# lxjeffffff/PagedAttention-Based-Transformer-Decoder-Inference-Framework

Hardware: AMD Instinct MI355X
Metric: decode tokens/sec at batch=64 seq_len=8192; % HBM-roofline (1/2/4/8 GPU) (higher is better)
Workload: dtype int8 GEMM (i32 acc) + fp16 KV attention (fp32 acc); 1 GPU; C3: INT8 decoder (MFMA i8 matmuls + fp16 paged attention), 24-layer/16-head/d=128, batch 64, KV context 8192, page 16; strong scaling: 64 rows over 1 GPU(s); global_batch=64, batch_per_gpu=64, seq_len=8192, page_size=16, parallelism=single GPU (no collective)

## Files before the change

pagedattention-based-transformer-decoder-inference-framework_amd/csrc/gemm_impl.hpp:

```cpp
#pragma once

#include "common.hpp"
#include "fp8.hpp"
#include "gemm.hpp"
#include "ln_wave.hpp"

namespace llm {

struct KvAppend {
  const int32_t* pos;
  const int32_t* page_table;
  const int32_t* rows;
  _Float16* k_pool;
  _Float16* v_pool;
  int num_beams, max_tiles, TS, num_pages, H, D;
  size_t page_stride;
  int fp8;
  float k_inv, v_inv;
};

struct GemmArgs {
  const uint8_t* A;
  int lda;
  int a_packed;
  const uint8_t* B;
  int M, N, K, KS;
  const float* sa;
  const float* sw;
  const float* bias;
  int act;
  float* C;
  int32_t* acc_out;
  int c_cols;
  int c_ld;
  _Float16* c16;
  KvAppend kv;
  unsigned long long* stamps;
  const float* ln_x;
  const _Float16* ln_emb;
  const int32_t* ln_tok;
  int ln_V;
  const float* ln_g;
  const float* ln_b;
  float ln_eps;
  uint8_t* act_out;
  float* sa_out;
  int partial;
  int w_keep;
  int xcd_map;
  unsigned* seam;
  int seam_n;
  int qdiag;
  int ksplit2;
};

__host__ __device__ constexpr int ln_row_stride(int K, int esize) { return K * esize + 32; }

__device__ __forceinline__ unsigned long long phase_clock() {
  unsigned long long t;
  asm volatile("s_memrealtime %0\n\ts_waitcnt lgkmcnt(0)" : "=s"(t)::"memory");
  return t;
}


template <int MT, int WAVES, int NT = 1>
constexpr int gemm_unroll() {
  return (MT >= 4 ? 2 : 4) * (WAVES == 4 ? 2 : 1) / (NT >= 4 ? 2 : 1);
}

__device__ __forceinline__ float apply_act(float y, int act) {
  if (act == LLM_ACT_RELU) return fmaxf(y, 0.f);
  if (act == LLM_ACT_GELU) return 0.5f * y * (1.f + erff(y * 0.70710678118654752f));
  return y;
}

enum class GemmKind { I8, F16 };

template <GemmKind KIND>
struct GemmTraits;
template <>
struct GemmTraits<GemmKind::I8> {
  static constexpr int KSTEP = 64, ESIZE = 1;
  using acc_t = i32x4;
  using elem_t = int32_t;
};
template <>
struct GemmTraits<GemmKind::F16> {
  static constexpr int KSTEP = 32, ESIZE = 2;
  using acc_t = f32x4;
  using elem_t = float;
};

template <GemmKind KIND, int ROWS, int WAVES>
__device__ __forceinline__ void ln_prologue(const GemmArgs& a, int m0, uint8_t* alds,
                                            float* sa_lds) {
  constexpr int ESIZE = GemmTraits<KIND>::ESIZE;
  constexpr int CPL = 8;
  const int lane = lane_id();
  const int w = wave_id_uniform();
  const int K = a.K;
  const int K4 = K >> 2;
  const int stride = ln_row_stride(K, ESIZE);
  const bool do_ln = a.ln_g != nullptr;
  LnRow<CPL> gm, bt;
  ln_wave_load(a.ln_g, K4, do_ln, gm);
  ln_wave_load(a.ln_b, K4, do_ln, bt);
  for (int r0 = w; r0 < ROWS; r0 += 2 * WAVES) {
    LnRow<CPL> x[2];
#pragma unroll
    for (int q = 0; q < 2; ++q) {
      const int r = r0 + q * WAVES;
      const int m = m0 + r;
      const bool ok = r < ROWS && m < a.M;
      if (a.ln_emb)
        ln_wave_load_f16(ok ? ln_embed_row(a.ln_emb, a.ln_tok, m, a.ln_V, K) : a.ln_emb, K4, ok,
// ... 5 lines not shown
    for (int q = 0; q < 2; ++q) {
      const int r = r0 + q * WAVES;
      if (r >= ROWS) break;
      const bool mok = m0 + r < a.M;
      float am;
      if (do_ln) {
        am = ln_wave_compute(x[q], gm, bt, K, a.ln_eps);
      } else {
        am = 0.f;
#pragma unroll
        for (int j = 0; j < CPL; ++j)
#pragma unroll
          for (int e = 0; e < 4; ++e) am = fmaxf(am, fabsf(x[q].v[j][e]));
        am = ln_wave_max(am);
      }
      uint8_t* rowp = alds + (size_t)r * stride;
      if constexpr (KIND == GemmKind::I8) {
        const float scale = 127.f / (am + 1e-6f);
#pragma unroll
        for (int j = 0; j < CPL; ++j) {
          const int c = 64 * j + lane;
          if (c < K4)
            *reinterpret_cast<uint32_t*>(rowp + 4 * c) = mok ? ln_quant4(x[q].v[j], scale) : 0u;
        }
        if (lane == 0) sa_lds[r] = mok ? 1.0f / scale : 0.f;
      } else {
#pragma unroll
        for (int j = 0; j < CPL; ++j) {
          const int c = 64 * j + lane;
          if (c < K4)
            *reinterpret_cast<ln_f16x4*>(rowp + 8 * c) =
                mok ? ln_half4(x[q].v[j]) : ln_f16x4{0, 0, 0, 0};
        }
      }
    }
  }
}

__device__ __forceinline__ void seam_wait(unsigned* ctr, int n) {
  if (threadIdx.x == 0) {
    unsigned spins = 0;
    while (__hip_atomic_load(&ctr[0], __ATOMIC_RELAXED, __HIP_MEMORY_SCOPE_AGENT) < (unsigned)n) {
      __builtin_amdgcn_s_sleep(8);
      if (++spins > (1u << 21)) {
        __hip_atomic_store(&ctr[2], 1u, __ATOMIC_RELAXED, __HIP_MEMORY_SCOPE_AGENT);
        break;
      }
    }
    __builtin_amdgcn_fence(__ATOMIC_ACQUIRE, "agent");
  }
  __syncthreads();
}

template <GemmKind KIND, int MT, int NT, int WAVES, int DIAG = 0, int PRO = 0, int SEAM = 0>
__device__ __forceinline__ void gemm_tile(const GemmArgs& a, int bx, int by, int bz, int nz,
                                          int gx) {
  using Tr = GemmTraits<KIND>;
  using acc_t = typename Tr::acc_t;
  constexpr int KSTEP = Tr::KSTEP;
  constexpr int kUnroll = gemm_unroll<MT, WAVES, NT>();
  using elem_t = typename Tr::elem_t;
  using RedT = elem_t[MT * NT][4][64];
  extern __shared__ __attribute__((aligned(16))) uint8_t gemm_smem[];
  RedT* red;
  if constexpr (PRO == 0) {
    __shared__ elem_t red_static[WAVES][MT * NT][4][64];
    red = red_static;
  } else {
    red = reinterpret_cast<RedT*>(gemm_smem);
  }
  constexpr int ROWS_ = 16 * MT;
  const int a_stride = ln_row_stride(a.K, Tr::ESIZE);
  uint8_t* alds = gemm_smem;
  float* sa_lds = reinterpret_cast<float*>(gemm_smem + (size_t)ROWS_ * a_stride);

  const int lane = lane_id();
  const int w = wave_id_uniform();
  const int nt0 = bx * NT;
  const int m0 = by * 16 * MT;
  unsigned long long* stamp =
      a.stamps ? a.stamps + ((size_t)by * gx + bx) * 48 : nullptr;
  if (stamp && lane == 0) stamp[w] = phase_clock();
  const int wr = (w + bx) % WAVES;
  const int kz0 = (int)((bz * a.KS) / nz);
  const int kzn = (int)(((bz + 1) * a.KS) / nz) - kz0;
  const int ks0 = kz0 + (wr * kzn) / WAVES;
  const int ks1 = kz0 + ((wr + 1) * kzn) / WAVES;
  const int ntiles = (a.N + 15) >> 4;

  const int arow_lane = lane & 15;
  const int kgrp = lane >> 4;
  const bool apk = a.a_packed;
  const uint32_t a_bytes = apk ? (uint32_t)(((a.M + 15) / 16) * a.KS * 1024u)
                               : (uint32_t)((size_t)a.M * a.lda * Tr::ESIZE);
  const auto arsrc = __builtin_amdgcn_make_buffer_rsrc((void*)a.A, (short)0, a_bytes, 0x00020000);
  const uint32_t a_kstride = apk ? 1024u : (uint32_t)(KSTEP * Tr::ESIZE);
  const uint32_t a_kgrp_off = apk ? 0u : (uint32_t)(kgrp * (KSTEP / 4) * Tr::ESIZE);
  uint32_t a_row_off[MT];
#pragma unroll
  for (int mt = 0; mt < MT; ++mt) {
    const int row = m0 + mt * 16 + arow_lane;
    a_row_off[mt] = row >= a.M ? 0xFFFFFFF0u
                    : apk ? (uint32_t)((((m0 >> 4) + mt) * a.KS) * 1024u + lane * 16)
                          : (uint32_t)((size_t)row * a.lda * Tr::ESIZE);
  }
  const uint8_t* bbase = a.B + (size_t)nt0 * a.KS * 1024;
  const uint32_t b_bytes = (uint32_t)(min(NT, ntiles - nt0) * a.KS * 1024u);
  uint32_t b_lane_off[NT];
#pragma unroll
  for (int j = 0; j < NT; ++j) b_lane_off[j] = (uint32_t)j * a.KS * 1024u + lane * 16;
  const auto brsrc = __builtin_amdgcn_make_buffer_rsrc((void*)bbase, (short)0, b_bytes, 0x00020000);

  acc_t acc[MT][NT];
#pragma unroll
  for (int mt = 0; mt < MT; ++mt)
#pragma unroll
    for (int j = 0; j < NT; ++j) acc[mt][j] = acc_t{0, 0, 0, 0};

  struct Batch {
    u32x4 b[kUnroll][NT];
    u32x4 af[kUnroll][MT];
  };
  auto issue = [&](Batch& bt, int ks, bool do_a = true, bool do_b = true) {
#pragma unroll
    for (int u = 0; u < kUnroll; ++u) {
      const int kk = ks + u;
      const bool ok = kk < ks1;
#pragma unroll
      for (int j = 0; j < NT; ++j) {
        if (!do_b) break;
        const uint32_t boff = ok ? b_lane_off[j] + (uint32_t)kk * 1024u : 0xFFFFFFF0u;
        bt.b[u][j] = a.w_keep ? __builtin_amdgcn_raw_buffer_load_b128(brsrc, boff, 0, 0)
                              : __builtin_amdgcn_raw_buffer_load_b128(brsrc, boff, 0, 2);
      }
// ... 51 lines not shown
    const int n = nt0 * 16 + o % COLS;
    const bool valid = o < ROWS * COLS && m < a.M && n < a.N;
    e_scale[e] = 1.f;
    if constexpr (KIND == GemmKind::I8) {
      if (!PRO && valid && a.sa) e_scale[e] *= a.sa[m];
      if (valid && a.sw) e_scale[e] *= a.sw[n];
    }
    e_bias[e] = valid && a.bias && (!a.ksplit2 || bz == 0) ? a.bias[n] : 0.f;
    const bool kvcol = valid && kv.k_pool && n >= hid;
    e_pos[e] = kvcol ? kv.pos[m] : -1;
    e_br[e] = kvcol ? (kv.rows ? kv.rows[m] : m) : -1;
  }

  Batch b0, b1;
  bool b1_pre = false;
  if constexpr (PRO != 0) {
    bool pre = true;
#if LLM_TUNING
    pre = (a.qdiag & 2) == 0;
#endif
    if (pre && ks0 < ks1) issue(b0, ks0, false, true);
    if (pre && ks0 + kUnroll < ks1) {
      issue(b1, ks0 + kUnroll, false, true);
      b1_pre = true;
    }
    if constexpr (SEAM != 0) seam_wait(a.seam, a.seam_n);
#if LLM_TUNING
    if ((a.qdiag & 1) == 0)
#endif
    ln_prologue<KIND, ROWS_, WAVES>(a, m0, alds, sa_lds);
    __syncthreads();
    if constexpr (KIND == GemmKind::I8) {
#pragma unroll
      for (int e = 0; e < EPT; ++e) {
        const int o = threadIdx.x + e * NTHR;
        if (o < ROWS * COLS) e_scale[e] *= sa_lds[o / COLS];
      }
    }
    if (a.act_out && bx == 0) {
      const int KS = a.KS;
      for (int i = threadIdx.x; i < ROWS_ * KS * 4; i += NTHR) {
        const int r = i / (KS * 4), g = i % (KS * 4);
        const int m = m0 + r;
        if (m >= a.M) continue;
        const size_t off = ((size_t)((m >> 4) * KS + (g >> 2)) * 64 + (m & 15) + 16 * (g & 3)) * 16;
        *reinterpret_cast<u32x4*>(a.act_out + off) =
            *reinterpret_cast<const u32x4*>(alds + (size_t)r * a_stride + 16 * g);
      }
      if (KIND == GemmKind::I8 && a.sa_out && threadIdx.x < ROWS_ && m0 + (int)threadIdx.x < a.M)
        a.sa_out[m0 + threadIdx.x] = sa_lds[threadIdx.x];
    }
  }

  {
    int ks = ks0;
    bool b0_b = PRO == 0;
#if LLM_TUNING
    if constexpr (PRO != 0) b0_b = (a.qdiag & 2) != 0;
#endif
    if (ks < ks1) issue(b0, ks, true, b0_b);
#pragma unroll
    for (int e = 0; e < EPT; ++e) {
      const int o = threadIdx.x + e * NTHR;
      const int n = nt0 * 16 + o % COLS;
      const int p = e_pos[e], br = e_br[e];
      int page = -1;
      if (p >= 0 && br >= 0 && br < kv.num_beams && p / kv.TS < kv.max_tiles) {
        const int which = n >= 2 * hid;
        const int h = (n - hid * (1 + which)) / kv.D;
        page = kv.page_table[((size_t)br * kv.H + h) * kv.max_tiles + p / kv.TS];
        if (page >= kv.num_pages) page = -1;
      }
      e_page[e] = page;
    }
    while (ks < ks1) {
      if (ks + kUnroll < ks1) {
        issue(b1, ks + kUnroll, true, !b1_pre);
        b1_pre = false;
      }
      compute(b0);
      ks += kUnroll;
      if (ks >= ks1) break;
      if (ks + kUnroll < ks1) issue(b0, ks + kUnroll);
      compute(b1);
      ks += kUnroll;
    }
  }

  if (stamp && lane == 0) stamp[16 + w] = phase_clock();
  if constexpr ((DIAG & 2) != 0) {
    int32_t x = 0;
#pragma unroll
    for (int mt = 0; mt < MT; ++mt)
#pragma unroll
      for (int j = 0; j < NT; ++j) x ^= (int32_t)acc[mt][j][0] ^ (int32_t)acc[mt][j][3];
    if (lane == 0 && a.C) a.C[bx] = (float)x;
    if (stamp && lane == 0) stamp[32 + w] = phase_clock();
    return;
  }
  if constexpr (PRO != 0) __syncthreads();
#pragma unroll
  for (int mt = 0; mt < MT; ++mt)
#pragma unroll
    for (int j = 0; j < NT; ++j)
#pragma unroll
      for (int r = 0; r < 4; ++r) red[wr][mt * NT + j][r][lane] = acc[mt][j][r];
  __syncthreads();

#pragma unroll
  for (int e = 0; e < EPT; ++e) {
#pragma clang fp contract(off)
    const int o = threadIdx.x + e * NTHR;
    if (o >= ROWS * COLS) break;
    const int cl = o % COLS;
    const int row = o / COLS;
    const int j = cl >> 4;
    const int col = cl & 15;
    const int mt = row >> 4;
    const int rl = row & 15;
    const int src_lane = (rl >> 2) * 16 + col;
    const int reg = rl & 3;
    const int m = m0 + row;
    const int n = (nt0 + j) * 16 + col;
    if (m >= a.M || n >= a.N) continue;
    float y;
    if constexpr (KIND == GemmKind::I8) {
      int32_t s = 0;
#pragma unroll
      for (int ww = 0; ww < WAVES; ++ww) s += red[ww][mt * NT + j][reg][src_lane];
#if LLM_TUNING
      if (a.partial) {
        a.acc_out[((size_t)bz * a.M + m) * a.N + n] = s;
        continue;
      }
#endif
      if (a.acc_out) a.acc_out[(size_t)m * a.N + n] = s;
      y = (float)s * e_scale[e];
      if (a.bias) y = y + e_bias[e];
      if (a.ksplit2) {
        atomicAdd(a.C + (size_t)m * a.c_ld + n, y);
        continue;
      }
    } else {
      float s = 0.f;
#pragma unroll
      for (int ww = 0; ww < WAVES; ++ww) s += red[ww][mt * NT + j][reg][src_lane];
      y = a.bias ? s + e_bias[e] : s;
    }
    y = apply_act(y, a.act);
    if (a.C && n < a.c_cols) a.C[(size_t)m * a.c_ld + n] = y;
    if (a.c16) a.c16[a_frag_off_f16(m, n, a.N >> 5)] = (_Float16)y;
    if (e_page[e] >= 0) {
      const int which = n >= 2 * hid;
      const int i = n - hid * (1 + which);
      const int d = i % kv.D;
      const int p = e_pos[e];
      const size_t off = (size_t)e_page[e] * kv.page_stride + (size_t)(p % kv.TS) * kv.D + d;
      if (kv.fp8)
        reinterpret_cast<uint8_t*>(which ? kv.v_pool : kv.k_pool)[off] =
            (uint8_t)fp8_e4m3_byte(y, which ? kv.v_inv : kv.k_inv);
      else
        (which ? kv.v_pool : kv.k_pool)[off] = (_Float16)y;
    }
  }
  if (stamp && lane == 0) stamp[32 + w] = phase_clock();
}

template <GemmKind KIND, int MT, int NT, int WAVES, int DIAG = 0, int PRO = 0>
__global__ __launch_bounds__(WAVES * 64) void gemm_kernel(GemmArgs a) {
  int bx = blockIdx.x, by = blockIdx.y, bz = blockIdx.z;
#if LLM_TUNING
  if (a.xcd_map) {
    const int per = 8 / (int)gridDim.z;
    const int lin = blockIdx.x + gridDim.x * (blockIdx.y + gridDim.y * blockIdx.z);
    const int xcd = lin & 7;
    const int tile = (lin >> 3) * per + xcd % per;
    bz = xcd / per;
    bx = tile % (int)gridDim.x;
    by = tile / (int)gridDim.x;
  }
#endif
  gemm_tile<KIND, MT, NT, WAVES, DIAG, PRO>(a, bx, by, bz, (int)gridDim.z, (int)gridDim.x);
}

template <typename T, int EPL>
__global__ void pack_kernel(const T* __restrict__ W, T* __restrict__ P, int K, int N, int KS,
                            int ntiles) {
  const size_t idx = (size_t)blockIdx.x * blockDim.x + threadIdx.x;
  const size_t total = (size_t)ntiles * KS * 64;
  if (idx >= total) return;
  const int lane = idx & 63;
  const size_t blk = idx >> 6;
  const int ks = blk % KS;
  const int nt = blk / KS;
  const int n = nt * 16 + (lane & 15);
  const int kb = ks * (4 * EPL) + (lane >> 4) * EPL;
  T* dst = P + idx * EPL;
#pragma unroll
  for (int j = 0; j < EPL; ++j) {
    const int k = kb + j;
    dst[j] = (k < K && n < N) ? W[(size_t)k * N + n] : T(0);
  }
}

namespace {

inline int pick_nt(int N, int M) {
  if (M <= 16) return 1;
  const int ntiles = (N + 15) / 16;
  const int mblocks = (M + 63) / 64;
  return (ntiles % 2 == 0 && (ntiles / 2) * mblocks >= 192) ? 2 : 1;
}

template <GemmKind KIND, int MT, int NT, int WAVES>
size_t ln_lds_bytes(int K) {
  const size_t img = (size_t)16 * MT * ln_row_stride(K, GemmTraits<KIND>::ESIZE) + 16 * MT * 4;
  const size_t red = (size_t)WAVES * MT * NT * 4 * 64 * 4;
  return img > red ? img : red;
}
constexpr size_t kLnLdsMax = 160 * 1024;

struct GemmForm {
  int mt;
  int nt;
  int waves;
  int kslices;
  int prologue;
};

template <GemmKind KIND, int MT, int NT>
hipError_t launch_gemm_nt(const GemmArgs& a, const GemmForm& f, int mblocks, hipStream_t st) {
  const int ntiles = (a.N + 15) / 16;
  const dim3 grid((ntiles + NT - 1) / NT, mblocks, f.kslices);
  if constexpr (NT <= 2) {
    if (f.prologue) {
      const size_t lds = ln_lds_bytes<KIND, MT, NT, 8>(a.K);
      hipLaunchKernelGGL((gemm_kernel<KIND, MT, NT, 8, 0, 1>), grid, dim3(512), lds, st, a);
      return hipGetLastError();
    }
  }
  if constexpr (MT * NT * 8 <= 64) {
    if (f.waves == 8) {
      hipLaunchKernelGGL((gemm_kernel<KIND, MT, NT, 8>), grid, dim3(512), 0, st, a);
      return hipGetLastError();
    }
  }
  hipLaunchKernelGGL((gemm_kernel<KIND, MT, NT, 4>), grid, dim3(256), 0, st, a);
  return hipGetLastError();
}

template <GemmKind KIND, int MT>
hipError_t launch_gemm_mt(const GemmArgs& a, const GemmForm& f, int mblocks, hipStream_t st) {
#if LLM_TUNING
  if (f.nt == 4) return launch_gemm_nt<KIND, MT, 4>(a, f, mblocks, st);
  if (f.nt == 3) return launch_gemm_nt<KIND, MT, 3>(a, f, mblocks, st);
#endif
  return f.nt == 2 ? launch_gemm_nt<KIND, MT, 2>(a, f, mblocks, st)
                   : launch_gemm_nt<KIND, MT, 1>(a, f, mblocks, st);
}

}

namespace {

inline int pick_waves(const GemmArgs&, int) { return 8; }

struct TileChoice {
  int nt, waves, mrows;
};
inline bool narrow_tile_for(int M, int N, int K, TileChoice& t) {
  if (M <= 16 || M > 64) return false;
  const int ntiles = (N + 15) / 16;
  if (M > 32) {
    if (ntiles >= 256) return false;
    t = TileChoice{2, 8, 16};
    return true;
  }
  if (ntiles < 384) {
    t = K >= 4096 ? TileChoice{1, 8, 16} : TileChoice{1, 4, 16};
    return true;
  }
  if (ntiles < 512) {
    t = TileChoice{1, 4, 16};
    return true;
  }
  return false;
}
inline bool narrow_decode_tile(const GemmArgs& a, int kstep, TileChoice& t) {
  if ((a.ln_x && a.ln_g) || a.partial) return false;
  if (a.ksplit2 && a.M > 32 && a.M <= 64) {
    t = TileChoice{2, 8, 64};
    return true;
  }
  return narrow_tile_for(a.M, a.N, a.KS * kstep, t);
}

inline GemmForm gemm_form(const GemmArgs& a, int kstep, int nt_override = 0,
                          int waves_override = 0, int mrows_override = 0, int ks_override = 0) {
  TileChoice tc{0, 0, 0};
  const bool narrow = nt_override == 0 && waves_override == 0 && mrows_override == 0 &&
                      narrow_decode_tile(a, kstep, tc);
  if (narrow) {
    nt_override = tc.nt;
    waves_override = tc.waves;
    mrows_override = tc.mrows;
  }
  const int NT = nt_override > 0 ? nt_override : pick_nt(a.N, a.M);
  const int waves = waves_override > 0 ? waves_override : pick_waves(a, NT);
  int mrows = a.M <= 16 ? 16 : a.M <= 32 ? 32 : 64;
  if (mrows == 64 && NT == 1 && (a.N + 15) / 16 < 256 && !a.ln_x && !a.partial) mrows = 32;
  if (mrows_override > 0) mrows = mrows_override;
  GemmForm f{};
  f.mt = mrows == 16 ? 1 : mrows == 32 ? 2 : 4;
  f.nt = NT == 2 ? 2 : 1;
#if LLM_TUNING
  if ((NT == 3 || NT == 4) && !a.ln_x) f.nt = NT;
#endif
  f.prologue = a.ln_x != nullptr;
  f.waves = f.prologue || (f.mt * f.nt * 8 <= 64 && waves != 4) ? 8 : 4;
  f.kslices = a.partial ? std::max(1, ks_override) : a.ksplit2 ? 2 : 1;
  return f;
}

template <GemmKind KIND>
hipError_t launch_gemm(const GemmArgs& a_in, hipStream_t st, int nt_override = 0,
                       int waves_override = 0, int mrows_override = 0, int ks_override = 0) {
  GemmArgs a = a_in;
  const GemmForm f = gemm_form(a, GemmTraits<KIND>::KSTEP, nt_override, waves_override,
                               mrows_override, ks_override);
  const int mblocks = (a.M + 16 * f.mt - 1) / (16 * f.mt);
  const int tiles = ((a.N + 15) / 16 + f.nt - 1) / f.nt * mblocks;
  if (a.xcd_map && (f.kslices < 2 || 8 % f.kslices != 0 || (tiles * f.kslices) % 8 != 0))
    a.xcd_map = 0;
  if (f.mt == 1) return launch_gemm_mt<KIND, 1>(a, f, mblocks, st);
  if (f.mt == 2) return launch_gemm_mt<KIND, 2>(a, f, mblocks, st);
  return launch_gemm_mt<KIND, 4>(a, f, mblocks, st);
}

}
}
```

pagedattention-based-transformer-decoder-inference-framework_amd/csrc/tune/gemm_tune.hip:

```cpp
#include "gemm_impl.hpp"

using namespace llm;

__global__ void gemm_end_stamp_kernel(unsigned long long* t) {
  if (threadIdx.x == 0) *t = phase_clock();
}

extern "C" int i8_gemm_stamps(int nt, int waves, int mrows, const int8_t* A, const void* W_packed,
                              float* C, int M, int N, int K, const float* sa, const float* sw,
                              unsigned long long* stamps, unsigned long long* end_stamp,
                              void* stream) {
  GemmArgs a{};
  a.a_packed = 1;
  a.A = reinterpret_cast<const uint8_t*>(A);
  a.lda = K;
  a.B = static_cast<const uint8_t*>(W_packed);
  a.M = M; a.N = N; a.K = K; a.KS = K / 64;
  a.sa = sa; a.sw = sw; a.C = C; a.c_cols = N; a.c_ld = N;
  a.stamps = stamps;
  hipStream_t st = as_stream(stream);
  hipError_t e = hipSuccess;
  const int ntiles = N / 16;
  const int diag = waves >> 8;
  if (diag == 0) {
    e = launch_gemm<GemmKind::I8>(a, st, nt, waves, mrows);
  } else {
    LLM_REQUIRE((nt == 2 && mrows == 64) || (nt == 1 && mrows == 32), "i8_gemm_stamps: diag shape");
    auto go = [&](auto kern, int NTv, int mr) {
      hipLaunchKernelGGL(kern, dim3((ntiles + NTv - 1) / NTv, (M + mr - 1) / mr), dim3(512), 0, st, a);
    };
    if (nt == 2) {
      if (diag == 1) go(gemm_kernel<GemmKind::I8, 4, 2, 8, 1>, 2, 64);
      else if (diag == 2) go(gemm_kernel<GemmKind::I8, 4, 2, 8, 2>, 2, 64);
      else go(gemm_kernel<GemmKind::I8, 4, 2, 8, 3>, 2, 64);
    } else {
      if (diag == 1) go(gemm_kernel<GemmKind::I8, 2, 1, 8, 1>, 1, 32);
      else if (diag == 2) go(gemm_kernel<GemmKind::I8, 2, 1, 8, 2>, 1, 32);
      else go(gemm_kernel<GemmKind::I8, 2, 1, 8, 3>, 1, 32);
    }
    e = hipGetLastError();
  }
  if (e == hipSuccess) {
    hipLaunchKernelGGL(gemm_end_stamp_kernel, dim3(1), dim3(64), 0, st, end_stamp);
    e = hipGetLastError();
  }
  return e == hipSuccess ? LLM_OK : fail(LLM_ERR_HIP, "i8_gemm_stamps");
}

extern "C" int i8_gemm_tune(int nt, int waves, int mrows, int a_packed, const int8_t* A, int lda,
                            const void* W_packed, float* C, int M, int N, int K, const float* sa,
                            const float* sw, void* stream) {
  GemmArgs a{};
  a.a_packed = a_packed;
  a.A = reinterpret_cast<const uint8_t*>(A);
  a.lda = lda;
  a.B = static_cast<const uint8_t*>(W_packed);
  a.M = M; a.N = N; a.K = K; a.KS = K / 64;
  a.sa = sa; a.sw = sw; a.C = C; a.c_cols = N; a.c_ld = N;
  hipError_t e = launch_gemm<GemmKind::I8>(a, as_stream(stream), nt, waves, mrows);
  return e == hipSuccess ? LLM_OK : fail(LLM_ERR_HIP, "i8_gemm_tune");
}

extern "C" int i8_gemm_tune_qpro(const float* x, const void* W_packed, float* C, int M, int N,
                                 int K, const float* sw, int qdiag, void* stream) {
  LLM_REQUIRE(quant_prologue_ok(M, N, K), "i8_gemm_tune_qpro: shape");
  GemmArgs a{};
  a.a_packed = 1;
  a.B = static_cast<const uint8_t*>(W_packed);
  a.M = M; a.N = N; a.K = K; a.KS = K / 64;
  a.sw = sw; a.C = C; a.c_cols = N; a.c_ld = N;
  a.ln_x = x;
  a.ln_eps = 1e-5f;
  a.qdiag = qdiag;
  hipError_t e = launch_gemm<GemmKind::I8>(a, as_stream(stream));
  return e == hipSuccess ? LLM_OK : fail(LLM_ERR_HIP, "i8_gemm_tune_qpro");
}

extern "C" int i8_gemm_tune_sk(int nt, int waves, int mrows, int kslices, int xcd_map,
                               const int8_t* A, const void* W_packed, int32_t* acc_out, int M,
                               int N, int K, void* stream) {
  LLM_REQUIRE(kslices >= 1 && kslices <= 8 && K % 64 == 0 && N % 16 == 0, "i8_gemm_tune_sk: shape");
  GemmArgs a{};
  a.a_packed = 1;
  a.A = reinterpret_cast<const uint8_t*>(A);
  a.lda = K;
  a.B = static_cast<const uint8_t*>(W_packed);
  a.M = M; a.N = N; a.K = K; a.KS = K / 64;
  a.partial = 1;
  a.acc_out = acc_out;
  a.xcd_map = xcd_map;
  hipError_t e = launch_gemm<GemmKind::I8>(a, as_stream(stream), nt, waves, mrows, kslices);
  return e == hipSuccess ? LLM_OK : fail(LLM_ERR_HIP, "i8_gemm_tune_sk");
}

__global__ __launch_bounds__(512) void gemm_pair_f16_kernel(GemmArgs a1, GemmArgs a2, int n1,
                                                            unsigned* sync) {
  const int wg = blockIdx.x;
  if (wg < n1) {
    gemm_tile<GemmKind::F16, 1, 1, 8, 0, 0>(a1, wg, 0, 0, 1, n1);
// ... 106 lines not shown
  kv.pos = t->kv_pos;
  kv.page_table = t->kv_page_table;
  kv.rows = t->kv_rows;
  kv.k_pool = t->kv_k_pool;
  kv.v_pool = t->kv_v_pool;
  kv.num_beams = t->kv_num_beams; kv.max_tiles = t->kv_max_tiles;
  kv.page_size = t->kv_page_size; kv.num_pages = t->kv_num_pages;
  kv.H = t->kv_H; kv.D = t->kv_D;
  kv.page_stride = (size_t)t->kv_page_stride;
  kv.kv_dtype = t->kv_dtype;
  kv.k_inv_scale = t->kv_k_inv_scale; kv.v_inv_scale = t->kv_v_inv_scale;
  WeightGemm g;
  g.dtype = t->dtype;
  g.A = t->A; g.lda = t->lda; g.a_packed = t->a_packed;
  g.W_packed = t->W_packed;
  g.M = t->M; g.N = t->N; g.K = t->K;
  g.sa = t->sa; g.sw = t->sw; g.bias = t->bias; g.act = t->act;
  g.C = t->C; g.c_cols = t->c_cols; g.c_ld = t->c_ld;
  g.C16 = t->C16;
  g.kv = t->has_kv ? &kv : nullptr;
  g.ln_x = t->ln_x;
  g.ln_emb = static_cast<const _Float16*>(t->ln_emb);
  g.ln_tok = t->ln_tok; g.ln_V = t->ln_V;
  g.ln_g = t->ln_g; g.ln_b = t->ln_b; g.ln_eps = t->ln_eps;
  g.act_out = t->act_out; g.sa_out = t->sa_out;
  g.w_keep = t->w_keep;
  g.ln_quant_only = t->ln_quant_only;
  g.ksplit2 = t->ksplit2;
  return weight_gemm(g, as_stream(stream));
}

extern "C" int gemm_ln_fusable_tune(int dtype, int M, int K) { return ln_fusable(dtype, M, K); }

extern "C" int gemm_quant_prologue_ok_tune(int M, int N, int K) {
  return quant_prologue_ok(M, N, K);
}

extern "C" int gemm_form_tune(int dtype, int M, int N, int K, int prologue, int ksplit2, int nt,
                              int waves, int mrows, int* form) {
  LLM_REQUIRE(form && M > 0 && N > 0 && K > 0 && (dtype == LLM_I8 || dtype == LLM_F16) &&
                  prologue >= 0 && prologue <= 2,
              "gemm_form_tune: bad arguments");
  const int kstep = dtype == LLM_I8 ? 64 : 32;
  static const float never_read = 0.f;
  GemmArgs a{};
  a.M = M; a.N = N; a.K = K; a.KS = K / kstep;
  a.ln_x = prologue ? &never_read : nullptr;
  a.ln_g = prologue == 1 ? &never_read : nullptr;
  a.ksplit2 = ksplit2;
  const GemmForm f = gemm_form(a, kstep, nt, waves, mrows);
  form[0] = f.mt; form[1] = f.nt; form[2] = f.waves; form[3] = f.kslices; form[4] = f.prologue;
  return LLM_OK;
}
```

pagedattention-based-transformer-decoder-inference-framework_amd/llm_capi.py:

```python
from __future__ import annotations

import ctypes
import os
from pathlib import Path

HERE = Path(__file__).resolve().parent
LIB_PATH = HERE / "libllm_decoder_hip.so"
TUNE_LIB_PATH = HERE / "libllm_decoder_hip_tune.so"

(LLM_OK, LLM_ERR_INVALID, LLM_ERR_UNSUPPORTED, LLM_ERR_HIP, LLM_ERR_OOM, LLM_ERR_IO,
 LLM_ERR_RANGE) = range(7)
LLM_F16, LLM_I8, LLM_F32, LLM_BF16, LLM_FP8 = 0, 1, 2, 3, 4
LLM_ACT_NONE, LLM_ACT_RELU, LLM_ACT_GELU = 0, 1, 2
LLM_EVICT_NONE, LLM_EVICT_LRU = 0, 1

c_int, c_float, c_void_p, c_size_t = ctypes.c_int, ctypes.c_float, ctypes.c_void_p, ctypes.c_size_t
c_ll = ctypes.c_longlong
c_i32p = ctypes.POINTER(ctypes.c_int32)


class PaKvView(ctypes.Structure):
    _fields_ = [("k_pool", c_void_p), ("v_pool", c_void_p), ("page_table", c_void_p),
                ("num_pages", ctypes.c_int32), ("page_size", ctypes.c_int32),
                ("head_dim", ctypes.c_int32), ("num_beams", ctypes.c_int32),
# ... 66 lines not shown
                                  c_void_p, c_int, c_int, c_int, c_int, c_float, c_int, c_int,
                                  c_void_p, c_size_t, c_void_p]),
    "pa_decode_ex": (c_int, [ctypes.POINTER(PaKvView), c_void_p, c_void_p, c_void_p, c_void_p,
                             c_int, c_int, c_int, c_int, ctypes.POINTER(PaDecodeOptions),
                             c_void_p, c_size_t, c_void_p]),
    "pa_prefill_workspace_bytes": (c_size_t, [ctypes.POINTER(PaKvView), c_int, c_int]),
    "pa_decode_ex_workspace_bytes": (c_size_t, [c_int, c_int, c_int]),
    "pa_prefill": (c_int, [ctypes.POINTER(PaKvView), c_void_p, c_int, c_void_p, c_int, c_int,
                           c_int, c_int, c_float, c_void_p, c_size_t, c_void_p]),
    "pa_prefill_packed_tiles": (c_int, [ctypes.POINTER(PaKvView), ctypes.POINTER(PaPrefillSeg),
                                        c_int, c_i32p, c_int]),
    "pa_prefill_packed_workspace_bytes": (c_size_t, [ctypes.POINTER(PaKvView),
                                                     ctypes.POINTER(PaPrefillSeg), c_int, c_int]),
    "pa_prefill_packed": (c_int, [ctypes.POINTER(PaKvView), c_void_p, c_int, c_void_p, c_int,
                                  ctypes.POINTER(PaPrefillSeg), c_int, c_float, c_void_p,
                                  c_size_t, c_void_p]),
    "llm_decoder_prefill_rows": (c_int, [c_void_p, c_i32p, c_i32p, c_i32p, c_int]),
    "llm_decoder_set_packed_prefill": (c_int, [c_void_p, c_int]),
    "llm_decoder_packed_prefill": (c_int, [c_void_p]),
    "gemm_packed_bytes": (c_size_t, [c_int, c_int, c_int]),
    "gemm_pack_weights": (c_int, [c_int, c_void_p, c_void_p, c_int, c_int, c_void_p]),
    "i8_gemm": (c_int, [c_void_p, c_int, c_void_p, c_void_p, c_void_p, c_int, c_int, c_int,
                        c_void_p, c_void_p, c_void_p, c_int, c_void_p]),
    "i8_matmul_s8": (c_int, [c_void_p, c_void_p, c_void_p, c_int, c_int, c_int, c_int, c_float,
                             c_float, c_float, c_void_p, c_int, c_void_p]),
    "f16_gemm": (c_int, [c_void_p, c_int, c_void_p, c_void_p, c_int, c_int, c_int, c_void_p,
                         c_int, c_void_p]),
    "lm_head": (c_int, [c_void_p, c_void_p, c_void_p, c_int, c_int, c_int, c_void_p]),
    "argmax_rows": (c_int, [c_void_p, c_int, c_int, c_void_p, c_void_p]),
    "sample_rows": (c_int, [c_void_p, c_int, c_int, c_float, c_int, c_float, ctypes.c_uint64,
                            c_int, c_void_p, c_void_p]),
    "sample_uniform_host": (c_float, [ctypes.c_uint64, c_int, c_int]),
    "beam_select_rows": (c_int, [c_void_p, c_void_p, c_int, c_int, c_int, c_void_p, c_void_p,
                                 c_void_p, c_void_p]),
    "kv_cache_reorder": (c_int, [c_void_p, c_int, c_int, c_i32p, c_int]),
    "kv_cache_cow_copies": (c_ll, [c_void_p]),
    "llm_decoder_beam_search": (c_int, [c_void_p, c_i32p, c_i32p, c_int, c_int,
                                        ctypes.POINTER(LlmBeamOptions), c_i32p, c_i32p,
                                        ctypes.POINTER(c_float), ctypes.POINTER(c_float)]),
    "quantize_rows": (c_int, [c_void_p, c_int, c_int, c_void_p, c_void_p, c_void_p]),
    "layernorm_quant": (c_int, [c_void_p, c_int, c_int, c_void_p, c_void_p, c_float, c_void_p,
                                c_void_p, c_void_p, c_void_p]),
    "layernorm_quant_tune": (c_int, [c_void_p, c_int, c_int, c_void_p, c_void_p, c_float, c_void_p,
                                     c_void_p, c_void_p, c_int, c_void_p, c_void_p, c_int,
                                     c_void_p, c_void_p]),
    "layernorm_f16_tune": (c_int, [c_void_p, c_int, c_int, c_void_p, c_void_p, c_float, c_void_p,
                                   c_int, c_void_p, c_void_p, c_int, c_void_p, c_void_p]),
    "quantize_rows_tune": (c_int, [c_void_p, c_int, c_int, c_void_p, c_void_p, c_int, c_void_p]),
    "to_f16_tune": (c_int, [c_void_p, c_size_t, c_void_p, c_int, c_void_p]),
    "weight_gemm_tune": (c_int, [ctypes.POINTER(WeightGemmTuneArgs), c_void_p]),
    "gemm_ln_fusable_tune": (c_int, [c_int, c_int, c_int]),
    "gemm_quant_prologue_ok_tune": (c_int, [c_int, c_int, c_int]),
    "gemm_form_tune": (c_int, [c_int] * 9 + [c_i32p]),
    "f16_gemm_tune": (c_int, [c_int] * 4 + [c_void_p, c_int, c_void_p, c_void_p] + [c_int] * 3 +
                      [c_void_p]),
    "kv_cache_create": (c_int, [c_int, c_int, c_int, c_int, c_int, c_int, c_ll,
                                ctypes.POINTER(c_void_p)]),
    "kv_cache_create_typed": (c_int, [c_int, c_int, c_int, c_int, c_int, c_int, c_ll, c_int,
                                      ctypes.POINTER(c_void_p)]),
    "kv_cache_destroy": (None, [c_void_p]),
    "kv_cache_view": (c_int, [c_void_p, c_int, ctypes.POINTER(PaKvView)]),
    "kv_cache_num_pages": (c_ll, [c_void_p]),
    "kv_cache_free_pages": (c_ll, [c_void_p]),
    "kv_cache_assign": (c_int, [c_void_p, c_int, c_int, c_int, c_int, c_int]),
    "kv_cache_lookup": (c_int, [c_void_p, c_int, c_int, c_int, c_int]),
    "kv_cache_remove": (c_int, [c_void_p, c_int, c_int, c_int, c_int]),
    "kv_cache_register_tile": (c_int, [c_void_p, c_int, c_int, c_int, c_int, c_i32p]),
    "kv_cache_set_eviction": (c_int, [c_void_p, c_int]),
    "kv_cache_reserve": (c_int, [c_void_p, c_int, c_int]),
    "kv_cache_fork": (c_int, [c_void_p, c_int, c_int]),
    "kv_cache_release": (c_int, [c_void_p, c_int]),
    "kv_cache_clear": (c_int, [c_void_p]),
    "kv_cache_sync": (c_int, [c_void_p, c_void_p]),
    "kv_cache_write_tokens": (c_int, [c_void_p, c_int, c_int, c_int, c_int, c_void_p, c_void_p]),
    "kv_cache_k_pool": (c_void_p, [c_void_p]),
    "kv_cache_v_pool": (c_void_p, [c_void_p]),
    "kv_cache_page_stride": (ctypes.c_longlong, [c_void_p]),
    "kv_cache_page_table": (c_void_p, [c_void_p, c_int]),
    "kv_cache_save": (c_int, [c_void_p, ctypes.c_char_p]),
    "kv_cache_load": (c_int, [c_void_p, ctypes.c_char_p]),
    "kv_cache_inspect": (c_int, [ctypes.c_char_p, ctypes.POINTER(ctypes.c_longlong)]),
    "kv_cache_save_pools": (c_int, [c_void_p, ctypes.c_char_p]),
    "kv_cache_load_pools": (c_int, [c_void_p, ctypes.c_char_p]),
    "kv_cache_save_tiles": (c_int, [c_void_p, c_int, c_int, ctypes.c_char_p]),
    "kv_cache_load_tiles": (c_int, [c_void_p, c_int, c_int, ctypes.c_char_p]),
    "kv_tiles_inspect": (c_int, [ctypes.c_char_p, ctypes.c_longlong, ctypes.POINTER(c_int)]),
    "llm_decoder_oproj_status": (c_int, [c_void_p, ctypes.POINTER(c_int),
                                         ctypes.POINTER(ctypes.c_longlong)]),
}

_lib = None


def declared_symbols() -> list[str]:
    import re
    hdr = (HERE.parent / "include" / "llm_decoder.h").read_text()
    hdr = re.sub(r"/\*.*?\*/", "", hdr, flags=re.S)
    names = re.findall(r"\b([a-z_][a-z0-9_]*)\s*\(", hdr)
    skip = {"if", "for", "while", "sizeof", "return", "defined"}
    return sorted({n for n in names if n not in skip})


def load(path: str | Path | None = None) -> ctypes.CDLL:
    global _lib
    if _lib is not None and path is None:
        return _lib
# ... 299 lines not shown
```

Baseline: 3797 tokens/s.

## Add whole-range streaming int8 GEMM path for narrow decode tiles

Adds a streaming variant of the int8 MFMA GEMM for single-row-tile, narrow-N decode shapes. Each wave issues all of its K-slice A and B buffer loads up front (depth 8 or 16) and then runs the MFMAs, replacing the double-buffered issue/compute loop. The goal is more memory-level parallelism on weight streaming at decode time. The cost is higher register pressure from holding FULL×NT 128-bit fragments per lane, which may reduce occupancy. Tuning hooks, extra stamps, and optional staggered walk orders are also added.

```diff
diff --git a/pagedattention-based-transformer-decoder-inference-framework_amd/csrc/gemm_impl.hpp b/pagedattention-based-transformer-decoder-inference-framework_amd/csrc/gemm_impl.hpp
--- a/pagedattention-based-transformer-decoder-inference-framework_amd/csrc/gemm_impl.hpp
+++ b/pagedattention-based-transformer-decoder-inference-framework_amd/csrc/gemm_impl.hpp
@@ -1,4 +1,6 @@
 #pragma once
+
+#include <type_traits>
 
 #include "common.hpp"
 #include "fp8.hpp"
@@ -61,6 +63,19 @@
   asm volatile("s_memrealtime %0\n\ts_waitcnt lgkmcnt(0)" : "=s"(t)::"memory");
   return t;
 }
+template <typename T>
+__device__ __forceinline__ unsigned long long phase_clock_after(T dep) {
+  unsigned long long t;
+  asm volatile("s_memrealtime %0\n\ts_waitcnt lgkmcnt(0)" : "=s"(t) : "v"(dep) : "memory");
+  return t;
+}
+constexpr int kGemmStampStride = 80;
+
+constexpr int kWalkStaggerA = 4, kWalkStaggerB = 8;
+constexpr int kStreamWalk = 0;
+constexpr bool stream_walk_valid(int w) {
+  return w == 0 || w == 1 || w == 2 || w == 4 || w == 5 || w == 12;
+}
 
 
 template <int MT, int WAVES, int NT = 1>
@@ -172,7 +187,8 @@
   __syncthreads();
 }
 
-template <GemmKind KIND, int MT, int NT, int WAVES, int DIAG = 0, int PRO = 0, int SEAM = 0>
+template <GemmKind KIND, int MT, int NT, int WAVES, int DIAG = 0, int PRO = 0, int SEAM = 0,
+          int FULL = 0, int WALK = 0>
 __device__ __forceinline__ void gemm_tile(const GemmArgs& a, int bx, int by, int bz, int nz,
                                           int gx) {
   using Tr = GemmTraits<KIND>;
@@ -199,7 +215,7 @@
   const int nt0 = bx * NT;
   const int m0 = by * 16 * MT;
   unsigned long long* stamp =
-      a.stamps ? a.stamps + ((size_t)by * gx + bx) * 48 : nullptr;
+      a.stamps ? a.stamps + ((size_t)by * gx + bx) * kGemmStampStride : nullptr;
   if (stamp && lane == 0) stamp[w] = phase_clock();
   const int wr = (w + bx) % WAVES;
   const int kz0 = (int)((bz * a.KS) / nz);
@@ -357,13 +373,7 @@
     }
   }
 
-  {
-    int ks = ks0;
-    bool b0_b = PRO == 0;
-#if LLM_TUNING
-    if constexpr (PRO != 0) b0_b = (a.qdiag & 2) != 0;
-#endif
-    if (ks < ks1) issue(b0, ks, true, b0_b);
+  auto lookup_pages = [&]() {
 #pragma unroll
     for (int e = 0; e < EPT; ++e) {
       const int o = threadIdx.x + e * NTHR;
@@ -378,16 +388,118 @@
       }
       e_page[e] = page;
     }
+  };
+  auto batch_stamp = [&](int bi) {
+#if LLM_TUNING
+    if (stamp && lane == 0 && w < 8 && bi < 4)
+      stamp[48 + 4 * w + bi] = phase_clock_after(acc[MT - 1][NT - 1][0]);
+#endif
+  };
+
+  if constexpr (FULL > 0) {
+    static_assert(KIND == GemmKind::I8 && MT == 1 && PRO == 0 && FULL % 4 == 0,
+                  "whole-range stream: exact int32 sums, one row tile, no prologue");
+    constexpr int ORDER = WALK & 3;
+    constexpr bool STAG_A = (WALK & kWalkStaggerA) != 0, STAG_B = (WALK & kWalkStaggerB) != 0;
+    u32x4 fb[FULL][NT], fa[FULL];
+    auto load_b = [&](int u, auto keep) {
+      const int kk = ks0 + u;
+#pragma unroll
+      for (int j = 0; j < NT; ++j) {
+        const uint32_t boff = kk < ks1 ? b_lane_off[j] + (uint32_t)kk * 1024u : 0xFFFFFFF0u;
+        if constexpr (decltype(keep)::value)
+          fb[u][j] = __builtin_amdgcn_raw_buffer_load_b128(brsrc, boff, 0, 0);
+        else
+          fb[u][j] = __builtin_amdgcn_raw_buffer_load_b128(brsrc, boff, 0, 2);
+      }
+      __builtin_amdgcn_sched_barrier(0);
+    };
+    const int a_end = a_row_off[0] != 0xFFFFFFF0u ? ks1 : ks0;
+    auto load_a = [&](int u) {
+      const int kk = ks0 + u;
+      const uint32_t koff = (uint32_t)kk * a_kstride + a_kgrp_off;
+      const uint32_t aoff = kk < a_end ? a_row_off[0] + koff : 0xFFFFFFF0u;
+      if constexpr ((DIAG & 1) != 0)
+        fa[u] = u32x4{aoff, 0u, 0u, 0u};
+      else
+        fa[u] = __builtin_amdgcn_raw_buffer_load_b128(arsrc, aoff, 0, 0);
+      __builtin_amdgcn_sched_barrier(0);
+    };
+    auto run = [&](auto rot, auto keep) {
+      constexpr int C = decltype(rot)::value;
+      constexpr int CA = STAG_A ? C : 0, CB = STAG_B ? C : 0;
+      constexpr int CM = ORDER == 1 ? CB : CA;
+      if constexpr (ORDER == 0) {
+#pragma unroll
+        for (int i = 0; i < FULL; ++i) load_b((i + CB) % FULL, keep);
+#pragma unroll
+        for (int i = 0; i < FULL; ++i) load_a((i + CA) % FULL);
+      } else if constexpr (ORDER == 1) {
+#pragma unroll
+        for (int i = 0; i < FULL; ++i) load_a((i + CA) % FULL);
+#pragma unroll
+        for (int i = 0; i < FULL; ++i) load_b((i + CB) % FULL, keep);
+      } else {
+#pragma unroll
+        for (int i = 0; i < FULL; ++i) {
+          load_b((i + CB) % FULL, keep);
+          load_a((i + CA) % FULL);
+        }
+      }
+      if (kv.k_pool) {
+        lookup_pages();
+      } else {
+#pragma unroll
+        for (int e = 0; e < EPT; ++e) e_page[e] = -1;
+      }
+#pragma unroll
+      for (int i = 0; i < FULL; ++i) {
+        const int u = (i + CM) % FULL;
+#pragma unroll
+        for (int j = 0; j < NT; ++j)
+          acc[0][j] = __builtin_amdgcn_mfma_i32_16x16x64_i8(__builtin_bit_cast(i32x4, fa[u]),
+                                                            __builtin_bit_cast(i32x4, fb[u][j]),
+                                                            acc[0][j], 0, 0, 0);
+        if ((i + 1) % (FULL / 4) == 0) batch_stamp(i / (FULL / 4));
+      }
+    };
+    auto run_rot = [&](auto rot) {
+      if (a.w_keep)
+        run(rot, std::true_type{});
+      else
+        run(rot, std::false_type{});
+    };
+    if constexpr (STAG_A || STAG_B) {
+      switch (((wr >> 2) + 2 * (by & 1)) & 3) {
+        case 0: run_rot(std::integral_constant<int, 0>{}); break;
+        case 1: run_rot(std::integral_constant<int, FULL / 4>{}); break;
+        case 2: run_rot(std::integral_constant<int, FULL / 2>{}); break;
+        default: run_rot(std::integral_constant<int, 3 * FULL / 4>{}); break;
+      }
+    } else {
+      run_rot(std::integral_constant<int, 0>{});
+    }
+  } else {
+    int ks = ks0;
+    bool b0_b = PRO == 0;
+#if LLM_TUNING
+    if constexpr (PRO != 0) b0_b = (a.qdiag & 2) != 0;
+#endif
+    if (ks < ks1) issue(b0, ks, true, b0_b);
+    lookup_pages();
+    int bi = 0;
     while (ks < ks1) {
       if (ks + kUnroll < ks1) {
         issue(b1, ks + kUnroll, true, !b1_pre);
         b1_pre = false;
       }
       compute(b0);
+      batch_stamp(bi++);
       ks += kUnroll;
       if (ks >= ks1) break;
       if (ks + kUnroll < ks1) issue(b0, ks + kUnroll);
       compute(b1);
+      batch_stamp(bi++);
       ks += kUnroll;
     }
   }
@@ -488,6 +600,12 @@
   gemm_tile<KIND, MT, NT, WAVES, DIAG, PRO>(a, bx, by, bz, (int)gridDim.z, (int)gridDim.x);
 }
 
+template <int NT, int FULL, int WALK, int DIAG = 0>
+__global__ __launch_bounds__(512) void gemm_stream_kernel(GemmArgs a) {
+  gemm_tile<GemmKind::I8, 1, NT, 8, DIAG, 0, 0, FULL, WALK>(a, blockIdx.x, blockIdx.y, 0, 1,
+                                                            (int)gridDim.x);
+}
+
 template <typename T, int EPL>
 __global__ void pack_kernel(const T* __restrict__ W, T* __restrict__ P, int K, int N, int KS,
                             int ntiles) {
@@ -508,6 +626,8 @@
   }
 }
 
+hipError_t launch_stream_gemm(int nt, int depth, const GemmArgs& a, dim3 grid, hipStream_t st);
+
 namespace {
 
 inline int pick_nt(int N, int M) {
@@ -531,7 +651,36 @@
   int waves;
   int kslices;
   int prologue;
+  int depth;
+  int walk;
 };
+
+template <int NT, int FULL, int DIAG = 0>
+hipError_t launch_gemm_stream(const GemmArgs& a, int walk, dim3 grid, hipStream_t st) {
+  auto go = [&](auto kern) {
+    hipLaunchKernelGGL(kern, grid, dim3(512), 0, st, a);
+    return hipGetLastError();
+  };
+  if (walk == kStreamWalk) {
+    if constexpr (DIAG == 0)
+      return launch_stream_gemm(NT, FULL, a, grid, st);
+    else
+      return go(gemm_stream_kernel<NT, FULL, kStreamWalk, DIAG>);
+  }
+#if LLM_TUNING
+  if constexpr (DIAG == 0 || NT == 2) {
+    switch (walk) {
+      case 0: return go(gemm_stream_kernel<NT, FULL, 0, DIAG>);
+      case 1: return go(gemm_stream_kernel<NT, FULL, 1, DIAG>);
+      case 2: return go(gemm_stream_kernel<NT, FULL, 2, DIAG>);
+      case 4: return go(gemm_stream_kernel<NT, FULL, 4, DIAG>);
+      case 5: return go(gemm_stream_kernel<NT, FULL, 5, DIAG>);
+      case 12: return go(gemm_stream_kernel<NT, FULL, 12, DIAG>);
+    }
+  }
+#endif
+  return hipErrorInvalidValue;
+}
 
 template <GemmKind KIND, int MT, int NT>
 hipError_t launch_gemm_nt(const GemmArgs& a, const GemmForm& f, int mblocks, hipStream_t st) {
@@ -543,6 +692,10 @@
       hipLaunchKernelGGL((gemm_kernel<KIND, MT, NT, 8, 0, 1>), grid, dim3(512), lds, st, a);
       return hipGetLastError();
     }
+  }
+  if constexpr (KIND == GemmKind::I8 && MT == 1 && NT <= 2) {
+    if (f.depth == 16) return launch_gemm_stream<NT, 16>(a, f.walk, grid, st);
+    if (f.depth == 8) return launch_gemm_stream<NT, 8>(a, f.walk, grid, st);
   }
   if constexpr (MT * NT * 8 <= 64) {
     if (f.waves == 8) {
@@ -600,8 +753,18 @@
   return narrow_tile_for(a.M, a.N, a.KS * kstep, t);
 }
 
+inline bool stream_form_ok(const GemmArgs& a, int kstep, const GemmForm& f) {
+  return kstep == 64 && f.mt == 1 && f.nt <= 2 && f.waves == 8 && !f.prologue && f.kslices == 1 &&
+         !a.partial && !a.ksplit2;
+}
+inline int stream_depth(int ksteps) {
+  const int per = (ksteps + 7) / 8;
+  return per > 16 ? 0 : per > 8 ? 16 : per > 4 ? 8 : 0;
+}
+
 inline GemmForm gemm_form(const GemmArgs& a, int kstep, int nt_override = 0,
-                          int waves_override = 0, int mrows_override = 0, int ks_override = 0) {
+                          int waves_override = 0, int mrows_override = 0, int ks_override = 0,
+                          int stream_override = -1) {
   TileChoice tc{0, 0, 0};
   const bool narrow = nt_override == 0 && waves_override == 0 && mrows_override == 0 &&
                       narrow_decode_tile(a, kstep, tc);
@@ -624,15 +787,29 @@
   f.prologue = a.ln_x != nullptr;
   f.waves = f.prologue || (f.mt * f.nt * 8 <= 64 && waves != 4) ? 8 : 4;
   f.kslices = a.partial ? std::max(1, ks_override) : a.ksplit2 ? 2 : 1;
+  if (stream_form_ok(a, kstep, f)) {
+    if (stream_override < 0) {
+      f.depth = narrow ? stream_depth(a.KS) : 0;
+      f.walk = f.depth ? kStreamWalk : 0;
+    } else {
+      f.depth = stream_override & 0xFF;
+      f.walk = f.depth ? stream_override >> 8 : 0;
+    }
+  }
   return f;
 }
 
 template <GemmKind KIND>
 hipError_t launch_gemm(const GemmArgs& a_in, hipStream_t st, int nt_override = 0,
-                       int waves_override = 0, int mrows_override = 0, int ks_override = 0) {
+                       int waves_override = 0, int mrows_override = 0, int ks_override = 0,
+                       int stream_override = -1) {
   GemmArgs a = a_in;
   const GemmForm f = gemm_form(a, GemmTraits<KIND>::KSTEP, nt_override, waves_override,
-                               mrows_override, ks_override);
+                               mrows_override, ks_override, stream_override);
+  if (f.depth && (!(f.depth == 8 || f.depth == 16) || (a.KS + 7) / 8 > f.depth ||
+                  !stream_walk_valid(f.walk)))
+    return hipErrorInvalidValue;
+  if (stream_override > 0 && !f.depth) return hipErrorInvalidValue;
   const int mblocks = (a.M + 16 * f.mt - 1) / (16 * f.mt);
   const int tiles = ((a.N + 15) / 16 + f.nt - 1) / f.nt * mblocks;
   if (a.xcd_map && (f.kslices < 2 || 8 % f.kslices != 0 || (tiles * f.kslices) % 8 != 0))
diff --git a/pagedattention-based-transformer-decoder-inference-framework_amd/csrc/stream_gemm.hip b/pagedattention-based-transformer-decoder-inference-framework_amd/csrc/stream_gemm.hip
--- /dev/null
+++ b/pagedattention-based-transformer-decoder-inference-framework_amd/csrc/stream_gemm.hip
@@ -0,0 +1,17 @@
+#include "gemm_impl.hpp"
+
+namespace llm {
+
+hipError_t launch_stream_gemm(int nt, int depth, const GemmArgs& a, dim3 grid, hipStream_t st) {
+  auto go = [&](auto kern) {
+    hipLaunchKernelGGL(kern, grid, dim3(512), 0, st, a);
+    return hipGetLastError();
+  };
+  if (nt == 2 && depth == 16) return go(gemm_stream_kernel<2, 16, kStreamWalk>);
+  if (nt == 2 && depth == 8) return go(gemm_stream_kernel<2, 8, kStreamWalk>);
+  if (nt == 1 && depth == 16) return go(gemm_stream_kernel<1, 16, kStreamWalk>);
+  if (nt == 1 && depth == 8) return go(gemm_stream_kernel<1, 8, kStreamWalk>);
+  return hipErrorInvalidValue;
+}
+
+}
diff --git a/pagedattention-based-transformer-decoder-inference-framework_amd/csrc/tune/gemm_tune.hip b/pagedattention-based-transformer-decoder-inference-framework_amd/csrc/tune/gemm_tune.hip
--- a/pagedattention-based-transformer-decoder-inference-framework_amd/csrc/tune/gemm_tune.hip
+++ b/pagedattention-based-transformer-decoder-inference-framework_amd/csrc/tune/gemm_tune.hip
@@ -6,10 +6,13 @@
   if (threadIdx.x == 0) *t = phase_clock();
 }
 
-extern "C" int i8_gemm_stamps(int nt, int waves, int mrows, const int8_t* A, const void* W_packed,
-                              float* C, int M, int N, int K, const float* sa, const float* sw,
-                              unsigned long long* stamps, unsigned long long* end_stamp,
-                              void* stream) {
+extern "C" int i8_gemm_stamps_stream(int nt, int waves, int mrows, int diag, int stream,
+                                     const int8_t* A, const void* W_packed, float* C, int M, int N,
+                                     int K, const float* sa, const float* sw,
+                                     unsigned long long* stamps, unsigned long long* end_stamp,
+                                     void* stream_ptr) {
+  LLM_REQUIRE(M > 0 && N > 0 && N % 16 == 0 && K > 0 && K % 64 == 0 && diag >= 0 && diag <= 3,
+              "i8_gemm_stamps: shape");
   GemmArgs a{};
   a.a_packed = 1;
   a.A = reinterpret_cast<const uint8_t*>(A);
@@ -18,18 +21,43 @@
   a.M = M; a.N = N; a.K = K; a.KS = K / 64;
   a.sa = sa; a.sw = sw; a.C = C; a.c_cols = N; a.c_ld = N;
   a.stamps = stamps;
-  hipStream_t st = as_stream(stream);
+  hipStream_t st = as_stream(stream_ptr);
   hipError_t e = hipSuccess;
   const int ntiles = N / 16;
-  const int diag = waves >> 8;
   if (diag == 0) {
-    e = launch_gemm<GemmKind::I8>(a, st, nt, waves, mrows);
+    e = launch_gemm<GemmKind::I8>(a, st, nt, waves, mrows, 0, stream);
+  } else if (mrows == 16) {
+    LLM_REQUIRE((nt == 1 || nt == 2) && waves == 8, "i8_gemm_stamps: diag shape");
+    const GemmForm f = gemm_form(a, 64, nt, waves, mrows, 0, stream);
+    LLM_REQUIRE(f.mt == 1 && f.nt == nt && f.waves == 8 &&
+                    (f.depth == 0 || ((a.KS + 7) / 8 <= f.depth && stream_walk_valid(f.walk))),
+                "i8_gemm_stamps: diag form");
+    const dim3 grid((ntiles + nt - 1) / nt, (M + 15) / 16);
+    auto narrow = [&](auto ntc, auto dc) {
+      constexpr int NTv = decltype(ntc)::value, D = decltype(dc)::value;
+      if (f.depth == 16) return launch_gemm_stream<NTv, 16, D>(a, f.walk, grid, st);
+      if (f.depth == 8) return launch_gemm_stream<NTv, 8, D>(a, f.walk, grid, st);
+      hipLaunchKernelGGL((gemm_kernel<GemmKind::I8, 1, NTv, 8, D>), grid, dim3(512), 0, st, a);
+      return hipGetLastError();
+    };
+    auto by_diag = [&](auto ntc) {
+      if (diag == 1) return narrow(ntc, std::integral_constant<int, 1>{});
+      if (diag == 2) return narrow(ntc, std::integral_constant<int, 2>{});
+      return narrow(ntc, std::integral_constant<int, 3>{});
+    };
+    e = nt == 2 ? by_diag(std::integral_constant<int, 2>{})
+                : by_diag(std::integral_constant<int, 1>{});
   } else {
-    LLM_REQUIRE((nt == 2 && mrows == 64) || (nt == 1 && mrows == 32), "i8_gemm_stamps: diag shape");
+    LLM_REQUIRE((nt == 2 && mrows == 64) || (nt == 1 && (mrows == 32 || mrows == 64)),
+                "i8_gemm_stamps: diag shape");
     auto go = [&](auto kern, int NTv, int mr) {
       hipLaunchKernelGGL(kern, dim3((ntiles + NTv - 1) / NTv, (M + mr - 1) / mr), dim3(512), 0, st, a);
     };
-    if (nt == 2) {
+    if (nt == 1 && mrows == 64) {
+      if (diag == 1) go(gemm_kernel<GemmKind::I8, 4, 1, 8, 1>, 1, 64);
+      else if (diag == 2) go(gemm_kernel<GemmKind::I8, 4, 1, 8, 2>, 1, 64);
+      else go(gemm_kernel<GemmKind::I8, 4, 1, 8, 3>, 1, 64);
+    } else if (nt == 2) {
       if (diag == 1) go(gemm_kernel<GemmKind::I8, 4, 2, 8, 1>, 2, 64);
       else if (diag == 2) go(gemm_kernel<GemmKind::I8, 4, 2, 8, 2>, 2, 64);
       else go(gemm_kernel<GemmKind::I8, 4, 2, 8, 3>, 2, 64);
@@ -45,6 +73,30 @@
     e = hipGetLastError();
   }
   return e == hipSuccess ? LLM_OK : fail(LLM_ERR_HIP, "i8_gemm_stamps");
+}
+
+extern "C" int i8_gemm_stamps(int nt, int waves, int mrows, const int8_t* A, const void* W_packed,
+                              float* C, int M, int N, int K, const float* sa, const float* sw,
+                              unsigned long long* stamps, unsigned long long* end_stamp,
+                              void* stream) {
+  return i8_gemm_stamps_stream(nt, waves & 0xFF, mrows, waves >> 8, -1, A, W_packed, C, M, N, K, sa,
+                               sw, stamps, end_stamp, stream);
+}
+
+extern "C" int i8_gemm_tune_stream(int nt, int waves, int mrows, int stream, const int8_t* A,
+                                   const void* W_packed, int32_t* acc_out, float* C, int M, int N,
+                                   int K, const float* sa, const float* sw, const float* bias,
+                                   void* stream_ptr) {
+  LLM_REQUIRE(M > 0 && N > 0 && N % 16 == 0 && K > 0 && K % 64 == 0, "i8_gemm_tune_stream: shape");
+  GemmArgs a{};
+  a.a_packed = 1;
+  a.A = reinterpret_cast<const uint8_t*>(A);
+  a.lda = K;
+  a.B = static_cast<const uint8_t*>(W_packed);
+  a.M = M; a.N = N; a.K = K; a.KS = K / 64;
+  a.sa = sa; a.sw = sw; a.bias = bias; a.C = C; a.acc_out = acc_out; a.c_cols = N; a.c_ld = N;
+  hipError_t e = launch_gemm<GemmKind::I8>(a, as_stream(stream_ptr), nt, waves, mrows, 0, stream);
+  return e == hipSuccess ? LLM_OK : fail(LLM_ERR_HIP, "i8_gemm_tune_stream");
 }
 
 extern "C" int i8_gemm_tune(int nt, int waves, int mrows, int a_packed, const int8_t* A, int lda,
@@ -257,3 +309,21 @@
   form[0] = f.mt; form[1] = f.nt; form[2] = f.waves; form[3] = f.kslices; form[4] = f.prologue;
   return LLM_OK;
 }
+
+extern "C" int gemm_form_stream_tune(int dtype, int M, int N, int K, int prologue, int ksplit2,
+                                     int nt, int waves, int mrows, int stream, int* form) {
+  LLM_REQUIRE(form && M > 0 && N > 0 && K > 0 && (dtype == LLM_I8 || dtype == LLM_F16) &&
+                  prologue >= 0 && prologue <= 2,
+              "gemm_form_stream_tune: bad arguments");
+  const int kstep = dtype == LLM_I8 ? 64 : 32;
+  static const float never_read = 0.f;
+  GemmArgs a{};
+  a.M = M; a.N = N; a.K = K; a.KS = K / kstep;
+  a.ln_x = prologue ? &never_read : nullptr;
+  a.ln_g = prologue == 1 ? &never_read : nullptr;
+  a.ksplit2 = ksplit2;
+  const GemmForm f = gemm_form(a, kstep, nt, waves, mrows, 0, stream);
+  form[0] = f.mt; form[1] = f.nt; form[2] = f.waves; form[3] = f.kslices; form[4] = f.prologue;
+  form[5] = f.depth; form[6] = f.walk;
+  return LLM_OK;
+}
diff --git a/pagedattention-based-transformer-decoder-inference-framework_amd/llm_capi.py b/pagedattention-based-transformer-decoder-inference-framework_amd/llm_capi.py
--- a/pagedattention-based-transformer-decoder-inference-framework_amd/llm_capi.py
+++ b/pagedattention-based-transformer-decoder-inference-framework_amd/llm_capi.py
@@ -142,6 +142,9 @@
     "gemm_ln_fusable_tune": (c_int, [c_int, c_int, c_int]),
     "gemm_quant_prologue_ok_tune": (c_int, [c_int, c_int, c_int]),
     "gemm_form_tune": (c_int, [c_int] * 9 + [c_i32p]),
+    "gemm_form_stream_tune": (c_int, [c_int] * 10 + [c_i32p]),
+    "i8_gemm_tune_stream": (c_int, [c_int] * 4 + [c_void_p] * 4 + [c_int] * 3 + [c_void_p] * 4),
+    "i8_gemm_stamps_stream": (c_int, [c_int] * 5 + [c_void_p] * 3 + [c_int] * 3 + [c_void_p] * 5),
     "f16_gemm_tune": (c_int, [c_int] * 4 + [c_void_p, c_int, c_void_p, c_void_p] + [c_int] * 3 +
                       [c_void_p]),
     "kv_cache_create": (c_int, [c_int, c_int, c_int, c_int, c_int, c_int, c_ll,
```

Result: no change. 3803 tokens/s, median of 6 (+0.2%).
